# kostas1515/object_detectors

Hardware: AMD Instinct MI355X
Metric: images/sec (fwd+bwd) YOLOv3 640px bs=32 (higher is better)
Workload: dtype bf16; 1 GPU; YOLOv3 Darknet-53 training step (fwd+loss+bwd+SGD step), synthetic COCO 640px, per-GPU bs=32, 7 GT/img, random-init weights; global_batch=32, parallelism=dp1

## Files before the change

### object_detectors_amd/build.py

```python
import os
import subprocess
import sys
from concurrent.futures import ThreadPoolExecutor

HERE = os.path.dirname(os.path.abspath(__file__))
CSRC = os.path.join(HERE, "csrc")
OBJ = os.path.join(CSRC, "build")
LIB = os.path.join(HERE, "libmi355det.so")
HIPCC = os.environ.get("HIPCC", "/opt/rocm/bin/hipcc")
ARCH = "gfx950"

SOURCES = [
    ("lib.cpp", []),
    ("yolo_kernels.hip", ["-ffp-contract=off"]),
    ("box_kernels.hip", ["-ffp-contract=off"]),
    ("roi_kernels.hip", ["-ffp-contract=off"]),
    ("proposal_kernels.hip", ["-ffp-contract=off"]),
    ("frcnn_kernels.hip", ["-ffp-contract=off"]),
    ("transform_kernels.hip", ["-ffp-contract=off"]),
    ("mask_kernels.hip", ["-ffp-contract=off"]),
    ("resnet_kernels.hip", []),
    ("conv_kernels.hip", []),
    ("igemm8_kernels.hip", []),
    ("wgrad_kernels.hip", []),
    ("dgrad_s2_kernels.hip", []),
    ("elem_kernels.hip", []),
    ("stem_kernels.hip", ["-fno-slp-vectorize"]),
    ("stem_l1_kernels.hip", ["-fno-slp-vectorize"]),
    ("rstem_kernels.hip", ["-fno-slp-vectorize"]),
]
F16_TWINS = ["conv_kernels.hip", "igemm8_kernels.hip", "wgrad_kernels.hip", "dgrad_s2_kernels.hip", "elem_kernels.hip", "stem_kernels.hip",
             "stem_l1_kernels.hip"]
COMMON = ["-O3", "-std=c++17", "-fPIC", f"--offload-arch={ARCH}", "-Wno-unused-value", "-x", "hip"]


def _stale(out, deps):
    if not os.path.exists(out):
        return True
    t = os.path.getmtime(out)
    return any(os.path.getmtime(d) > t for d in deps)


def build(force=False, verbose=False):
    os.makedirs(OBJ, exist_ok=True)
    headers = [os.path.join(CSRC, f) for f in os.listdir(CSRC) if f.endswith(".h")]
    headers.append(os.path.join(HERE, "..", "include", "mi355det.h"))
    jobs, objs = [], []
    for src, extra in SOURCES:
        sp = os.path.join(CSRC, src)
        if not os.path.exists(sp):
            raise FileNotFoundError(sp)
        op = os.path.join(OBJ, os.path.splitext(src)[0] + ".o")
        objs.append(op)
        if force or _stale(op, [sp] + headers):
            jobs.append([HIPCC] + COMMON + extra + ["-c", sp, "-o", op])
        if src in F16_TWINS:
            op16 = os.path.join(OBJ, os.path.splitext(src)[0] + "_f16.o")
            objs.append(op16)
            if force or _stale(op16, [sp] + headers):
                jobs.append([HIPCC] + COMMON + extra + ["-DMI355_F16=1", "-c", sp, "-o", op16])

    def run(cmd):
        if verbose:
            print(" ".join(cmd), flush=True)
# ... 15 lines not shown
```

### object_detectors_amd/csrc/conv_kernels.hip

```cpp
#include "common.h"

#include <cstdlib>

#include <unordered_map>

#include "tune_record.h"

using namespace mi355;

#include "igemm_common.h"

extern int g_wgrad_general;
extern int g_wgrad_force_dbg;
extern int g_wgrad8_off;
extern int g_wgrad_ablate;
extern int g_dgrad_s2_off;
extern int g_conv_strict;
int mi355det_internal_dgrad_s2(const mi355det_conv_shape* s, const void* dy, const void* wt, void* dx, const void* residual, int32_t residual_ld,
                               void* stream, int probe = 0);

namespace {

#define STAMP(v) do { if (PROF) { __builtin_amdgcn_sched_barrier(0); asm volatile("s_memtime %0\n\ts_waitcnt lgkmcnt(0)" : "=s"(v) :: "memory"); __builtin_amdgcn_sched_barrier(0); } } while (0)

template <int WM, int WN, int TM, int TN, int BK, int NST, int EPI, bool PROF = false, bool ILV = false, int OCC = 0, int ABL = 0>
__global__ __launch_bounds__(WM* WN * 64, (OCC > 0 ? OCC : (WM * WN >= 8 ? 2 : 1))) void igemm_kernel(const IgemmParams p) {
  unsigned long long t_a = 0, t_b = 0, t_c = 0, t_d = 0, t_e = 0, c_wait = 0, c_bar = 0, c_issue = 0, c_comp = 0, t_begin = 0, t_loop = 0;
  STAMP(t_begin);
  constexpr int NT = WM * WN * 64;
  constexpr int NW = WM * WN;
  constexpr int BM = WM * TM * 16, BN = WN * TN * 16;
  constexpr int ROWB = BK * 2;
  constexpr int R = 1024 / ROWB;
  constexpr int CPR = BK / 8;
  constexpr int A_INSTR = BM / R, B_INSTR = BN / R;
  constexpr int A_PER = (A_INSTR + NW - 1) / NW, B_PER = (B_INSTR + NW - 1) / NW;
  constexpr int PER = A_PER + B_PER;
  constexpr int STAGE = (BM + BN) * ROWB;
  constexpr int D = NST - 1;
  static_assert(A_INSTR % NW == 0, "A tile must split evenly over the waves");
  extern __shared__ __attribute__((aligned(16))) char smem[];
  int* s_toff = (int*)(smem + NST * STAGE);

  const int tid = threadIdx.x, lane = tid & 63;
  const int wid = __builtin_amdgcn_readfirstlane(tid >> 6);
  const int wm = wid % WM, wn = wid / WM;

// ... 947 lines not shown
    if (ms < best_ms) {
      best_ms = ms;
      best = cfg;
    }
  }
  g_igemm_tuned[igemm_key(p, EPI)] = best;
  tune_mark_timed(TUNE_IGEMM, igemm_key(p, EPI));
  static const bool tune_log = getenv("MI355DET_TUNE_LOG") != nullptr;
  if (tune_log) fprintf(stderr, "[mi355det] igemm tune: M=%d Cout=%d Cin=%d T=%d epi=%d -> cfg %d (%.1f us)\n", p.M, p.CoutPad, p.Cin, p.T, EPI, best, best_ms * 1e3f / 3.f);
  return best;
}

__global__ __launch_bounds__(256) void lattice_fill_kernel(bf16_t* __restrict__ dx, int ld, const bf16_t* __restrict__ res, int ldres, int n, int h, int w,
                                                            int mh, int mw, int py, int px, int c) {
  const int c8 = c / 8;
  const long long total = (long long)n * mh * mw * c8;
  for (long long i = (long long)blockIdx.x * blockDim.x + threadIdx.x; i < total; i += (long long)gridDim.x * blockDim.x) {
    const int ch = (int)(i % c8);
    long long t = i / c8;
    const int xx = (int)(t % mw);
    t /= mw;
    const int yy = (int)(t % mh), im = (int)(t / mh);
    const int oy = 2 * yy + py, ox = 2 * xx + px;
    if (oy >= h || ox >= w) continue;
    const long long pix = ((long long)im * h + oy) * w + ox;
    uint4 v = make_uint4(0, 0, 0, 0);
    if (res) v = *(const uint4*)(res + pix * ldres + ch * 8);
    *(uint4*)(dx + pix * ld + ch * 8) = v;
  }
}

bool g_autotune_mode = false;
TuneMap& g_s2cat_tuned = tune_table(TUNE_S2CAT);
int g_s2cat_force = -1;

template <int EPI>
int dispatch_igemm(const IgemmParams& p_in, hipStream_t st) {
  IgemmParams p = p_in;
  p.lin_in = p.T == 1 && p.dy[0] == 0 && p.dx[0] == 0 && p.sin == 1 && p.MH == p.Hin && p.MW == p.Win;
  p.lin_out = p.so == 1 && p.sox == 0 && p.oy0 == 0 && p.ox0 == 0 && p.MH == p.Hout && p.MW == p.Wout;
  return g_autotune_mode ? autotune_igemm<EPI>(p, st) : launch_igemm<EPI>(p, st);
}

void set_tap_pad(IgemmParams& p) {
  int mn = 0;
  p.dy_pack = p.dx_pack = 0;
  for (int t = 0; t < p.T; ++t) {
    mn = min(mn, (p.dy[t] * p.Win + p.dx[t]) * p.ldin);
    p.dy_pack |= (unsigned long long)(p.dy[t] + 2) << (4 * t);
    p.dx_pack |= (unsigned long long)(p.dx[t] + 2) << (4 * t);
  }
  p.tap_pad = -mn;
}

int check_shape(const mi355det_conv_shape* s, const char* what) {
  if (!s) return fail(MI355DET_EINVAL, "%s: null shape", what);
  if (!((s->ksize == 1 && s->pad == 0) || (s->ksize == 3 && s->pad == 1)) || (s->stride != 1 && s->stride != 2))
    return fail(MI355DET_EINVAL, "%s: only 1x1/p0 and 3x3/p1 with stride 1 or 2 are supported", what);
  if (s->ho != (s->h + 2 * s->pad - s->ksize) / s->stride + 1 || s->wo != (s->w + 2 * s->pad - s->ksize) / s->stride + 1)
    return fail(MI355DET_EINVAL, "%s: output size does not match the convolution geometry", what);
  if (s->in_ld < s->cin || s->out_ld < s->cout) return fail(MI355DET_EINVAL, "%s: pixel pitch smaller than channel count", what);
  return 0;
}

int grid_m_rows(const mi355det_conv_shape* s, int cout_pad) {
  (void)cout_pad;
  const int bm = 128;
  const long long M = (long long)s->n * s->ho * s->wo;
  return (int)((M + bm - 1) / bm);
}

}

extern "C" {

int mi355det_debug_set(int key, int value) {
  if (key == 0) g_tune = value;
  if (key == 1) g_wgrad_general = value;
  if (key == 2) g_dgrad_s2_off = value;
  if (key == 3) igemm8_set_dbg_mode(value);
  if (key == 8) g_wgrad8_off = value;
  if (key == 7) g_wgrad_force_dbg = value;
  if (key == 6) g_wgrad_ablate = value;
  if (key == 5) g_s2cat_force = value;
  if (key == 9) g_conv_strict = value;
  return 0;
}

int mi355det_conv_autotune_mode(int on) {
  g_autotune_mode = on != 0;
  return 0;
}

int mi355det_debug_ptr(int key, void* ptr) {
  if (key == 0) g_dbg = (unsigned long long*)ptr;
  if (key == 1) igemm8_set_dbg((unsigned long long*)ptr);
  return 0;
}

int mi355det_conv_stats_rows(const mi355det_conv_shape* s, int32_t cout_pad) {
  if (!s) return 0;
  return grid_m_rows(s, cout_pad);
}

static int conv_fwd_impl(const mi355det_conv_shape* s, const void* x, const void* w, const float* bias, void* y, int out_f32, float* stats,
                         int32_t cout_pad, const mi355det_conv_epilogue* ex, void* stream) {
  if (int e = check_shape(s, "conv_fwd")) return e;
  if (int e = ensure_zero_page()) return e;
  if (cout_pad < s->cout) return fail(MI355DET_EINVAL, "%s: cout_pad < cout", "conv_fwd");
  if (!out_f32 && (s->cout % 8)) return fail(MI355DET_EINVAL, "%s: 16-bit outputs need cout %% 8 == 0 (got %lld)", "conv_fwd", s->cout);
  IgemmParams p{};
  p.x = (const bf16_t*)x;
  p.w = (const bf16_t*)w;
  p.y = y;
  p.bias = bias;
  p.stats = stats;
  p.zero = g_zero_page;
// ... 555 lines not shown
```

### object_detectors_amd/csrc/f16_names.h

```cpp
#pragma once
#define mi355det_conv_autotune_mode mi355det_conv_autotune_mode_f16
#define mi355det_conv_dgrad mi355det_conv_dgrad_f16
#define mi355det_conv_dgrad_bn mi355det_conv_dgrad_bn_f16
#define mi355det_conv_dgrad_bn_rows mi355det_conv_dgrad_bn_rows_f16
#define mi355det_conv_dgrad_mask mi355det_conv_dgrad_mask_f16
#define mi355det_conv_dgrad_workspace mi355det_conv_dgrad_workspace_f16
#define mi355det_conv_dgrad_ws mi355det_conv_dgrad_ws_f16
#define mi355det_conv_fwd mi355det_conv_fwd_f16
#define mi355det_conv_fwd_ex mi355det_conv_fwd_ex_f16
#define mi355det_conv_stats_rows mi355det_conv_stats_rows_f16
#define mi355det_debug_ptr mi355det_debug_ptr_f16
#define mi355det_debug_set mi355det_debug_set_f16
#define mi355det_dgrad_pack_elems mi355det_dgrad_pack_elems_f16
#define mi355det_pack_table_build mi355det_pack_table_build_f16
#define mi355det_pack_table_bytes mi355det_pack_table_bytes_f16
#define mi355det_pack_weights mi355det_pack_weights_f16
#define mi355det_pack_weights_batched mi355det_pack_weights_batched_f16
#define mi355det_stem_im2col mi355det_stem_im2col_f16
#define mi355det_unpack_wgrad mi355det_unpack_wgrad_f16
#define mi355det_conv_wgrad mi355det_conv_wgrad_f16
#define mi355det_conv_wgrad_autotune mi355det_conv_wgrad_autotune_f16
#define mi355det_conv_wgrad_workspace mi355det_conv_wgrad_workspace_f16
#define mi355det_add_bf16 mi355det_add_bf16_f16
#define mi355det_bn_act_bwd_apply mi355det_bn_act_bwd_apply_f16
#define mi355det_bn_act_bwd_reduce mi355det_bn_act_bwd_reduce_f16
#define mi355det_bn_act_bwd_reduce_det mi355det_bn_act_bwd_reduce_det_f16
#define mi355det_bn_act_bwd_reduce_workspace mi355det_bn_act_bwd_reduce_workspace_f16
#define mi355det_bn_act_fwd mi355det_bn_act_fwd_f16
#define mi355det_nchw_f32_to_nhwc mi355det_nchw_f32_to_nhwc_f16
#define mi355det_nhwc_to_nchw_f32 mi355det_nhwc_to_nchw_f32_f16
#define mi355det_upsample2x_bwd mi355det_upsample2x_bwd_f16
#define mi355det_upsample2x_fwd mi355det_upsample2x_fwd_f16
#define mi355det_stem_bwd_apply_wgrad mi355det_stem_bwd_apply_wgrad_f16
#define mi355det_stem_bwd_finish mi355det_stem_bwd_finish_f16
#define mi355det_stem_bwd_fused mi355det_stem_bwd_fused_f16
#define mi355det_stem_bwd_reduce mi355det_stem_bwd_reduce_f16
#define mi355det_stem_fwd_apply mi355det_stem_fwd_apply_f16
#define mi355det_stem_fwd_stats mi355det_stem_fwd_stats_f16
#define mi355det_stem_rows mi355det_stem_rows_f16
#define mi355det_stem_l1_fwd mi355det_stem_l1_fwd_f16
#define mi355det_stem_l1_fwd_eval mi355det_stem_l1_fwd_eval_f16
#define mi355det_stem_l1_rows mi355det_stem_l1_rows_f16
#define mi355det_internal_dgrad_s2 mi355det_internal_dgrad_s2_f16
#define igemm8_launch igemm8_launch_f16
#define igemm8_set_dbg igemm8_set_dbg_f16
#define igemm8_applicable igemm8_applicable_f16
#define igemm8_set_dbg_mode igemm8_set_dbg_mode_f16
#define g_wgrad_general g_wgrad_general_f16
#define g_wgrad_force_dbg g_wgrad_force_dbg_f16
#define g_conv_strict g_conv_strict_f16
#define g_wgrad8_off g_wgrad8_off_f16
#define g_wgrad_ablate g_wgrad_ablate_f16
#define g_dgrad_s2_off g_dgrad_s2_off_f16
#define pack_batched_kernel pack_batched_kernel_f16
#define splitk_reduce_kernel splitk_reduce_kernel_f16
```

### object_detectors_amd/csrc/igemm_common.h

```cpp
#pragma once
#include "common.h"

using namespace mi355;

typedef __attribute__((ext_vector_type(4))) float f32x4_t;
typedef __attribute__((ext_vector_type(8))) unsigned short u16x8_t;

#define MAX_TAPS 9

struct FastDiv {
  unsigned mul, shift;
};
static FastDiv make_fastdiv(unsigned d) {
  FastDiv f;
  unsigned l = 0;
  while ((1ull << l) < d) ++l;
  f.shift = l;
  f.mul = (unsigned)(((1ull << 32) * ((1ull << l) - d)) / d + 1);
  return f;
}
__device__ __forceinline__ unsigned fdiv(unsigned n, const FastDiv f) { return (__umulhi(f.mul, n) + n) >> f.shift; }

struct IgemmParams {
  const bf16_t* x;
// ... 5 lines not shown
  long long ynstride;
  const bf16_t* z;
  const float* ss;
  int ldz;
  float slope;
  float* stats;
  const bf16_t* res;
  const bf16_t* zero;
  int M, MH, MW;
  int Hin, Win, ldin, Cin, sin;
  int Hout, Wout, ldout, so, oy0, ox0;
  int sox;
  int Cout, CoutPad, ldres;
  int T;
  int dy[MAX_TAPS], dx[MAX_TAPS];
  FastDiv dMW, dMH;
  int tap_pad;
  unsigned long long dy_pack, dx_pack;
  int ksplit;
  long long ysplit;
  int lin_in, lin_out;
  unsigned long long* dbg;
};

enum { EPI_STATS = 0, EPI_F32 = 1, EPI_RES = 2, EPI_PLAIN = 3, EPI_AFF = 4, EPI_BNRED = 5 };
#define EPI_LDS_OFF 4096
#define EPI_LDS_BYTES(nwaves) (EPI_LDS_OFF + (nwaves) * (64 * (8 * 16 * 2 + 16) + 256))

bool igemm8_applicable(const IgemmParams& p);
int igemm8_launch(int epi, const IgemmParams& p, hipStream_t st, int rows = 256);
void igemm8_set_dbg(unsigned long long* ptr);
void igemm8_set_dbg_mode(int mode);

namespace {

__device__ __forceinline__ void glds16(const void* gsrc, void* lds_dst_uniform) {
  __builtin_amdgcn_global_load_lds((const __attribute__((address_space(1))) void*)gsrc,
                                   (__attribute__((address_space(3))) void*)lds_dst_uniform, 16, 0, 0);
}

typedef __attribute__((ext_vector_type(4))) int srd_t;
__device__ __forceinline__ srd_t make_srd(const void* base, unsigned num_records) {
  const unsigned long long a = (unsigned long long)base;
  srd_t r;
  r[0] = (int)(unsigned)a;
  r[1] = (int)((unsigned)(a >> 32) & 0xFFFFu);
  r[2] = (int)num_records;
  r[3] = 0x00020000;
  return r;
}
__device__ __forceinline__ void bufld16(srd_t rsrc, const void* lds_dst_uniform, int voffset, int soffset) {
  const unsigned lds = (unsigned)(unsigned long long)(__attribute__((address_space(3))) const void*)lds_dst_uniform;
  asm volatile("s_mov_b32 m0, %0\n\ts_nop 0\n\tbuffer_load_dwordx4 %1, %2, %3 offen lds" ::"s"(lds), "v"(voffset), "s"(rsrc), "s"(soffset) : "memory");
}
#define OOB_VOFF ((int)0x80000000)

__device__ __forceinline__ float row16_sum(float v) {
  v += __builtin_bit_cast(float, __builtin_amdgcn_update_dpp(0, __builtin_bit_cast(int, v), 0xB1, 0xF, 0xF, true));
  v += __builtin_bit_cast(float, __builtin_amdgcn_update_dpp(0, __builtin_bit_cast(int, v), 0x4E, 0xF, 0xF, true));
  v += __builtin_bit_cast(float, __builtin_amdgcn_update_dpp(0, __builtin_bit_cast(int, v), 0x141, 0xF, 0xF, true));
  v += __builtin_bit_cast(float, __builtin_amdgcn_update_dpp(0, __builtin_bit_cast(int, v), 0x140, 0xF, 0xF, true));
  return v;
}

template <int BK>
__device__ __forceinline__ int swz(int row) {
// ... 307 lines not shown
```

### object_detectors_amd/csrc/wgrad_kernels.hip

```cpp
#include "common.h"

#include <cstdlib>
#include <unordered_map>

#include "tune_record.h"

using namespace mi355;

typedef __attribute__((ext_vector_type(4))) short s16x4_t;
typedef __attribute__((ext_vector_type(4))) float f32x4_t;

struct FastDiv {
  unsigned mul, shift, d;
};

static FastDiv make_fastdiv(unsigned d) {
  FastDiv f;
  f.d = d;
  unsigned l = 0;
  while ((1ull << l) < d) ++l;
  f.shift = l;
  f.mul = (unsigned)(((1ull << 32) * ((1ull << l) - d)) / d + 1);
  return f;
}
__device__ __forceinline__ unsigned fdiv(unsigned n, const FastDiv f) {
  const unsigned t = __umulhi(f.mul, n);
  return (t + n) >> f.shift;
}

struct WgradParams {
  const bf16_t* x;
  const bf16_t* dy;
  float* dw;
  float* slab;
  const bf16_t* zero;
  int M, Ho, Wo, H, W, ldx, lddy, Cin, Cout, stride, pad, ks, T, NP;
  int co_tiles, np_tiles, splits, chunk;
  int step_q, step_r;
  FastDiv dWo, dHo, dCin;
  int ablate;
};

int g_wgrad_ablate = 0;
int g_wgrad_general = 0;
int g_conv_strict = 0;
int g_wgrad_force_dbg = 0;
int g_wgrad8_off = 0;

namespace {

#define WG_BKP 64
#define WG_TILE 128
#define WG_ROWB 256

__device__ __forceinline__ void glds16(const void* gsrc, void* lds_dst_uniform) {
  __builtin_amdgcn_global_load_lds((const __attribute__((address_space(1))) void*)gsrc,
                                   (__attribute__((address_space(3))) void*)lds_dst_uniform, 16, 0, 0);
}

typedef __attribute__((ext_vector_type(4))) int srd_t;
__device__ __forceinline__ srd_t make_srd(const void* base, unsigned num_records) {
  const unsigned long long a = (unsigned long long)base;
  srd_t r;
  r[0] = (int)(unsigned)a;
  r[1] = (int)((unsigned)(a >> 32) & 0xFFFFu);
  r[2] = (int)num_records;
  r[3] = 0x00020000;
  return r;
}
__device__ __forceinline__ void bufld16(srd_t rsrc, const void* lds_dst_uniform, int voffset, int soffset) {
  const unsigned lds = (unsigned)(unsigned long long)(__attribute__((address_space(3))) const void*)lds_dst_uniform;
  asm volatile("s_mov_b32 m0, %0\n\ts_nop 0\n\tbuffer_load_dwordx4 %1, %2, %3 offen lds" ::"s"(lds), "v"(voffset), "s"(rsrc), "s"(soffset) : "memory");
}
#define OOB_VOFF ((int)0x80000000)

__device__ __forceinline__ int rowf(int row) { return (row & 3) | (((row >> 3) & 1) << 2); }

__device__ __forceinline__ st16x4_t lds_tr(const char* p) {
  s16x4_t v = __builtin_amdgcn_ds_read_tr16_b64_v4i16((__attribute__((address_space(3))) s16x4_t*)p);
// ... 522 lines not shown

  const int fr = lane & 15, fq = lane >> 4;
  const int nt128 = NT * 2 + wm;
  if (nt128 >= p.np_tiles) return;
  if (p.slab) {
    const int tiles = p.co_tiles * p.np_tiles;
#pragma unroll
    for (int a = 0; a < 4; ++a) {
      const int col = wn * 64 + (a >> 1) * 32 + (a & 1) * 16;
      const int ct128 = CT * 2 + (col >> 7);
      if (ct128 >= p.co_tiles) continue;
      float* dst = p.slab + ((size_t)split * tiles + (size_t)nt128 * p.co_tiles + ct128) * (WG_TILE * WG_TILE);
#pragma unroll
      for (int r = 0; r < 4; ++r)
#pragma unroll
        for (int b = 0; b < 8; ++b) dst[((col & 127) + fq * 4 + r) * WG_TILE + (b >> 2) * 64 + (b & 3) * 16 + fr] = acc[a][b][r];
    }
    return;
  }
#pragma unroll
  for (int a = 0; a < 4; ++a)
#pragma unroll
    for (int r = 0; r < 4; ++r) {
      const int co = co0 + wn * 64 + (a >> 1) * 32 + (a & 1) * 16 + fq * 4 + r;
      if (co >= p.Cout) continue;
#pragma unroll
      for (int b = 0; b < 8; ++b) {
        const int np = np0 + wm * 128 + (b >> 2) * 64 + (b & 3) * 16 + fr;
        if (np < p.NP) p.dw[(long long)co * p.NP + np] += acc[a][b][r];
      }
    }
}

__global__ __launch_bounds__(256) void wgrad_reduce_kernel(const float* __restrict__ slab, float* __restrict__ dw, int Cout, int NP, int co_tiles,
                                                           int np_tiles, int splits) {
  const int tiles = co_tiles * np_tiles;
  const long long total = (long long)Cout * (NP / 4);
  const size_t sstride = (size_t)tiles * (WG_TILE * WG_TILE);
  for (long long i = blockIdx.x * 256ll + threadIdx.x; i < total; i += (long long)gridDim.x * 256) {
    const int co = (int)(i / (NP / 4)), np = (int)(i - (long long)co * (NP / 4)) * 4;
    const int ct = co / WG_TILE, nt = np / WG_TILE;
    const int tile = nt * co_tiles + ct;
    const float* src = slab + (size_t)tile * (WG_TILE * WG_TILE) + (co - ct * WG_TILE) * WG_TILE + (np - nt * WG_TILE);
    float4 a = make_float4(0.f, 0.f, 0.f, 0.f);
    for (int s0 = blockIdx.y * 8; s0 < splits; s0 += gridDim.y * 8) {
      float4 v[8];
#pragma unroll
      for (int u = 0; u < 8; ++u) v[u] = s0 + u < splits ? *(const float4*)(src + (size_t)(s0 + u) * sstride) : make_float4(0.f, 0.f, 0.f, 0.f);
#pragma unroll
      for (int u = 0; u < 8; ++u) {
        a.x += v[u].x; a.y += v[u].y; a.z += v[u].z; a.w += v[u].w;
      }
    }
    float* d = dw + (long long)co * NP + np;
    if (gridDim.y == 1) {
      float4 o = *(const float4*)d;
      o.x += a.x; o.y += a.y; o.z += a.z; o.w += a.w;
      *(float4*)d = o;
    } else {
      atomicAdd(d + 0, a.x); atomicAdd(d + 1, a.y); atomicAdd(d + 2, a.z); atomicAdd(d + 3, a.w);
    }
  }
}

__global__ __launch_bounds__(256) void wgrad_reduce8_kernel(const float* __restrict__ slab, float* __restrict__ dw, int Cout, int NP, int co_tiles,
                                                            int np_tiles, int splits) {
// ... 176 lines not shown
}

TuneMap& g_wgrad_tuned = tune_table(TUNE_WGRAD);
int g_wgrad_force = 0;
constexpr int WG_FORM8 = 1 << 16;

unsigned long long wgrad_key(const mi355det_conv_shape* s) {
  unsigned long long k = (unsigned long long)(s->n * s->ho * s->wo);
  k = k * 4099 + s->cout;
  k = k * 4099 + s->cin;
  k = k * 17 + s->ksize * 4 + s->stride;
  k = k * 2 + MI355_F16;
  return k;
}

bool split_valid(int M, int sp) {
  const int chunk = ((M + sp - 1) / sp + WG_BKP - 1) / WG_BKP * WG_BKP;
  return (M + chunk - 1) / chunk == sp;
}

bf16_t* g_zero_page_w = nullptr;
int ensure_zero_page_w() {
  if (g_zero_page_w) return 0;
  void* p = nullptr;
  if (hipMalloc(&p, 4096) != hipSuccess || hipMemset(p, 0, 4096) != hipSuccess) return fail(MI355DET_ELAUNCH, "%s: zero page alloc failed", "wgrad");
  g_zero_page_w = (bf16_t*)p;
  return 0;
}

bool wgrad8_applicable(const mi355det_conv_shape* s) {
  const long long NP = (long long)s->ksize * s->ksize * s->cin;
  if (s->wo < 4 || WG_BKP / s->wo + 1 > s->ho || s->cout < 256 || NP < 256 || s->cin % 8 != 0) return false;
  return ((long long)s->n * s->h * s->w + (long long)s->pad * (s->w + 1)) * s->in_ld * 2 < 0x7FFFFFF0ll;
}

}

extern "C" {

size_t mi355det_conv_wgrad_workspace(const mi355det_conv_shape* s) {
  if (!s) return 0;
  const size_t tiles = (size_t)((s->cout + WG_TILE - 1) / WG_TILE) * (size_t)((s->ksize * s->ksize * s->cin + WG_TILE - 1) / WG_TILE);
  const size_t per_split = tiles * WG_TILE * WG_TILE * sizeof(float);
  size_t splits = 1024;
  while (splits > 3 && splits * per_split > ((size_t)128 << 20)) --splits;
  return splits * per_split;
}

int mi355det_conv_wgrad_autotune(const mi355det_conv_shape* s, const void* x, const void* dy, float* dw, void* workspace,
                                 size_t workspace_bytes, void* stream) {
  if (!s) return fail(MI355DET_EINVAL, "%s: null shape", "wgrad_autotune");
  if (tune_locked_has(TUNE_WGRAD, wgrad_key(s))) return g_wgrad_tuned[wgrad_key(s)];
  const int M = s->n * s->ho * s->wo;
  const size_t tiles = (size_t)((s->cout + WG_TILE - 1) / WG_TILE) * (size_t)((s->ksize * s->ksize * s->cin + WG_TILE - 1) / WG_TILE);
  const size_t per_split = tiles * WG_TILE * WG_TILE * sizeof(float);
  const int cands[] = {1, 2, 3, 4, 5, 6, 7, 8, 10, 12, 14, 16, 20, 24, 28, 32, 40, 48, 56, 64, 96, 128, 192, 256, 384, 512, 768, 1024};
  hipEvent_t e0, e1;
  if (hipEventCreate(&e0) != hipSuccess || hipEventCreate(&e1) != hipSuccess) return fail(MI355DET_ELAUNCH, "%s: event create failed", "wgrad_autotune");
  int best = -1;
  float best_ms = 1e30f;
  int tried[32], n_tried = 0;
  float tried_ms[32];
  for (int sp : cands) {
    if (sp > 1 && (sp * per_split > workspace_bytes || M / sp < 512 || (size_t)sp * tiles > 4096)) continue;
    if (!split_valid(M, sp)) continue;
    g_wgrad_force = sp;
// ... 118 lines not shown
    form8 = form8 && wgrad8_applicable(s);
    const size_t per_split = (size_t)tiles * WG_TILE * WG_TILE * sizeof(float);
    while (splits > 1 && (splits * per_split > workspace_bytes || !split_valid(p.M, splits))) --splits;
  }
  int chunk = (p.M + splits - 1) / splits;
  chunk = (chunk + WG_BKP - 1) / WG_BKP * WG_BKP;
  splits = (p.M + chunk - 1) / chunk;
  p.splits = splits;
  p.chunk = chunk;
  p.slab = nullptr;
  if (splits > 1) {
    const size_t need = (size_t)splits * tiles * WG_TILE * WG_TILE * sizeof(float);
    if (!workspace || workspace_bytes < need) return fail(MI355DET_EWORKSPACE, "%s: workspace too small (%lld bytes needed)", "conv_wgrad", (long long)need);
    if (p.NP % 4 != 0) return fail(MI355DET_EINVAL, "%s: k*k*Cin must be a multiple of 4", "conv_wgrad");
    p.slab = (float*)workspace;
  }
  p.step_q = WG_BKP / p.Wo;
  p.step_r = WG_BKP % p.Wo;
  p.dWo = make_fastdiv((unsigned)p.Wo);
  p.dHo = make_fastdiv((unsigned)p.Ho);
  p.dCin = make_fastdiv((unsigned)p.Cin);
  const int lds = 2 * 2 * WG_BKP * WG_ROWB;
  const int ci = p.Cout <= 32 ? 1 : (p.Cout <= 64 ? 2 : 4), cj = p.NP <= 32 ? 1 : (p.NP <= 64 ? 2 : 4);
  auto go = [&](auto kern) {
    (void)hipFuncSetAttribute((const void*)kern, hipFuncAttributeMaxDynamicSharedMemorySize, lds);
    hipLaunchKernelGGL(kern, dim3(tiles * splits), dim3(256), lds, S(stream), p);
  };
  const int grp4 = g_wgrad_general != 0 || p.Wo < 4 || WG_BKP / p.Wo + 1 > p.Ho ? 0 : (p.Wo % 16 == 0 ? 3 : (p.Wo % 4 == 0 ? 1 : 2));
  const bool fits =
                    ((long long)s->n * p.H * p.W + (long long)p.pad * (p.W + 1)) * p.ldx * 2 < 0x7FFFFFF0ll &&
                    (long long)chunk * p.lddy * 2 < 0x7FFFFFF0ll;
  if (form8 && !fits && g_conv_strict && g_wgrad_force <= 0 && (g_wgrad_force_dbg & WG_FORM8))
    return fail(MI355DET_EINVAL, "%s: the forced phase-staggered kernel does not fit the 31-bit offsets of this shape (strict mode, debug key 9)", "conv_wgrad");
  if (form8 && fits) {
    const int tiles8 = ((p.Cout + W8_TILE - 1) / W8_TILE) * ((p.NP + W8_TILE - 1) / W8_TILE);
    static DeviceOnce attr8;
    attr8.once([&] {
      (void)hipFuncSetAttribute((const void*)wgrad8_kernel<false>, hipFuncAttributeMaxDynamicSharedMemorySize, W8_LDS);
      (void)hipFuncSetAttribute((const void*)wgrad8_kernel<true>, hipFuncAttributeMaxDynamicSharedMemorySize, W8_LDS);
    });
    if (p.Wo % 4 == 0 && p.M % 4 == 0) hipLaunchKernelGGL(wgrad8_kernel<false>, dim3(tiles8 * splits), dim3(512), W8_LDS, S(stream), p);
    else hipLaunchKernelGGL(wgrad8_kernel<true>, dim3(tiles8 * splits), dim3(512), W8_LDS, S(stream), p);
  } else
#define WG_GO(a, b) (!fits || grp4 == 0 ? go(wgrad_kernel<a, b, 0>) : grp4 == 1 ? go(wgrad_kernel<a, b, 1>) : grp4 == 2 ? go(wgrad_kernel<a, b, 2>) : go(wgrad_kernel<a, b, 3>))
  switch (ci * 8 + cj) {
    case 1 * 8 + 1: WG_GO(1, 1); break;
    case 1 * 8 + 2: WG_GO(1, 2); break;
    case 1 * 8 + 4: WG_GO(1, 4); break;
    case 2 * 8 + 1: WG_GO(2, 1); break;
    case 2 * 8 + 2: WG_GO(2, 2); break;
    case 2 * 8 + 4: WG_GO(2, 4); break;
    case 4 * 8 + 1: WG_GO(4, 1); break;
    case 4 * 8 + 2: WG_GO(4, 2); break;
    default: WG_GO(4, 4); break;
  }
#undef WG_GO
  if (p.slab) {
    const long long total = (long long)p.Cout * (p.NP / 4);
    if (splits >= 8) {
      const int gx = (int)min((long long)4096, (total + 31) / 32);
      hipLaunchKernelGGL(wgrad_reduce8_kernel, dim3(gx), dim3(256), 0, S(stream), p.slab, dw, p.Cout, p.NP, p.co_tiles, p.np_tiles, splits);
    } else {
      const int gx = (int)min((long long)2048, (total + 255) / 256);
      hipLaunchKernelGGL(wgrad_reduce_kernel, dim3(gx, 1), dim3(256), 0, S(stream), p.slab, dw, p.Cout, p.NP, p.co_tiles, p.np_tiles, splits);
    }
  }
  if (dbias) {
// ... 20 lines not shown
```

Measured before the change: 1157 images/s.

## Add row-streaming 3x3 conv kernel with register-resident weights for small-channel layers

Adds a new implicit-GEMM kernel for 3x3 stride-1 convolutions with small channel counts. Each block keeps all of its filter weights in registers and streams input rows through an LDS ring buffer. Output rows are written one step late so stores overlap the next step's loads. By default it handles only the Cin=64, Cout=32 case at 320 width (the Darknet-53 first residual block), in both the forward and flipped-tap paths. BN statistics are reduced per strip into the existing row-partial layout. The aim is to cut redundant halo and input reloads in a bandwidth-bound layer, at the cost of low occupancy (one block per CU, large LDS footprint) and more code paths.

Result: no change. 1158 images/s, median of 4 (+0.1%).

```diff
diff --git a/object_detectors_amd/build.py b/object_detectors_amd/build.py
--- a/object_detectors_amd/build.py
+++ b/object_detectors_amd/build.py
@@ -22,6 +22,7 @@
     ("resnet_kernels.hip", []),
     ("conv_kernels.hip", []),
     ("igemm8_kernels.hip", []),
+    ("rowstream_kernels.hip", []),
     ("wgrad_kernels.hip", []),
     ("dgrad_s2_kernels.hip", []),
     ("elem_kernels.hip", []),
@@ -29,7 +30,7 @@
     ("stem_l1_kernels.hip", ["-fno-slp-vectorize"]),
     ("rstem_kernels.hip", ["-fno-slp-vectorize"]),
 ]
-F16_TWINS = ["conv_kernels.hip", "igemm8_kernels.hip", "wgrad_kernels.hip", "dgrad_s2_kernels.hip", "elem_kernels.hip", "stem_kernels.hip",
+F16_TWINS = ["conv_kernels.hip", "igemm8_kernels.hip", "rowstream_kernels.hip", "wgrad_kernels.hip", "dgrad_s2_kernels.hip", "elem_kernels.hip", "stem_kernels.hip",
              "stem_l1_kernels.hip"]
 COMMON = ["-O3", "-std=c++17", "-fPIC", f"--offload-arch={ARCH}", "-Wno-unused-value", "-x", "hip"]
 
diff --git a/object_detectors_amd/csrc/conv_kernels.hip b/object_detectors_amd/csrc/conv_kernels.hip
--- a/object_detectors_amd/csrc/conv_kernels.hip
+++ b/object_detectors_amd/csrc/conv_kernels.hip
@@ -1026,6 +1026,7 @@
 
 bool g_autotune_mode = false;
 TuneMap& g_s2cat_tuned = tune_table(TUNE_S2CAT);
+int g_rowstream_mode = 0;
 int g_s2cat_force = -1;
 
 template <int EPI>
@@ -1033,6 +1034,8 @@
   IgemmParams p = p_in;
   p.lin_in = p.T == 1 && p.dy[0] == 0 && p.dx[0] == 0 && p.sin == 1 && p.MH == p.Hin && p.MW == p.Win;
   p.lin_out = p.so == 1 && p.sox == 0 && p.oy0 == 0 && p.ox0 == 0 && p.MH == p.Hout && p.MW == p.Wout;
+  if ((EPI == EPI_STATS || EPI == EPI_PLAIN) && g_rowstream_mode != 1 && g_tune == 0 && rowstream_applicable(p, EPI, g_rowstream_mode >= 2))
+    return rowstream_launch(EPI, p, st, g_rowstream_mode >= 3 ? g_rowstream_mode - 2 : 0);
   return g_autotune_mode ? autotune_igemm<EPI>(p, st) : launch_igemm<EPI>(p, st);
 }
 
@@ -1077,6 +1080,7 @@
   if (key == 7) g_wgrad_force_dbg = value;
   if (key == 6) g_wgrad_ablate = value;
   if (key == 5) g_s2cat_force = value;
+  if (key == 10) g_rowstream_mode = value;
   if (key == 9) g_conv_strict = value;
   return 0;
 }
diff --git a/object_detectors_amd/csrc/f16_names.h b/object_detectors_amd/csrc/f16_names.h
--- a/object_detectors_amd/csrc/f16_names.h
+++ b/object_detectors_amd/csrc/f16_names.h
@@ -46,6 +46,8 @@
 #define igemm8_set_dbg igemm8_set_dbg_f16
 #define igemm8_applicable igemm8_applicable_f16
 #define igemm8_set_dbg_mode igemm8_set_dbg_mode_f16
+#define rowstream_applicable rowstream_applicable_f16
+#define rowstream_launch rowstream_launch_f16
 #define g_wgrad_general g_wgrad_general_f16
 #define g_wgrad_force_dbg g_wgrad_force_dbg_f16
 #define g_conv_strict g_conv_strict_f16
diff --git a/object_detectors_amd/csrc/igemm_common.h b/object_detectors_amd/csrc/igemm_common.h
--- a/object_detectors_amd/csrc/igemm_common.h
+++ b/object_detectors_amd/csrc/igemm_common.h
@@ -61,6 +61,9 @@
 void igemm8_set_dbg(unsigned long long* ptr);
 void igemm8_set_dbg_mode(int mode);
 
+bool rowstream_applicable(const IgemmParams& p, int epi, bool all = false);
+int rowstream_launch(int epi, const IgemmParams& p, hipStream_t st, int strip_rows = 0);
+
 namespace {
 
 __device__ __forceinline__ void glds16(const void* gsrc, void* lds_dst_uniform) {
diff --git a/object_detectors_amd/csrc/rowstream_kernels.hip b/object_detectors_amd/csrc/rowstream_kernels.hip
--- /dev/null
+++ b/object_detectors_amd/csrc/rowstream_kernels.hip
@@ -0,0 +1,296 @@
+#include "igemm_common.h"
+
+namespace {
+
+constexpr int RS_ROW_BYTES = 21 * 1024;
+constexpr int RS_PIECES = 21;
+constexpr int RS_WAVES = 4;
+constexpr int RS_TPW = 5;
+
+struct RowstreamParams {
+  const bf16_t* x;
+  const bf16_t* w;
+  bf16_t* y;
+  float* stats;
+  int N, H, W, ldin, ldout, Cout, CoutPad;
+  int R;
+  int nstrips, ncol, ncs;
+  int flip;
+  int M;
+};
+
+template <int CIN>
+__device__ __forceinline__ int rs_swz(int s) {
+  return CIN == 32 ? ((s >> 1) & 3) : (s & 7);
+}
+
+template <int CIN, int NWC, int PX, int EPI>
+__global__ __launch_bounds__(RS_WAVES * 64, 1) void rowstream_kernel(const RowstreamParams p) {
+  static_assert(CIN == 32 || CIN == 64, "one or two k-steps of 32 per tap");
+  static_assert(NWC % 32 == 0, "output channels in pairs of 16-row tiles");
+  static_assert(320 % PX == 0 && PX % 80 == 0, "a step is 320 pixels; a wave's five tiles lie in one row");
+  constexpr int PB = CIN * 2;
+  constexpr int CPP = PB / 16;
+  constexpr int KS = CIN / 32;
+  constexpr int NT = NWC / 16;
+  constexpr int NP = NT / 2;
+  constexpr int RS = 320 / PX;
+  constexpr int NR = 2 * RS + 2;
+  constexpr int TPR = PX / 16;
+  constexpr int NPW = (RS_PIECES + RS_WAVES - 1) / RS_WAVES;
+  static_assert((PX + 2) * PB <= RS_ROW_BYTES, "ring row pitch");
+  extern __shared__ __attribute__((aligned(16))) char smem[];
+
+  const int tid = threadIdx.x, lane = tid & 63;
+  const int wid = __builtin_amdgcn_readfirstlane(tid >> 6);
+  const int fr = lane & 15, fq = lane >> 4;
+
+  int bid = blockIdx.x;
+  const int cs = bid % p.ncs;
+  bid /= p.ncs;
+  const int cc = bid % p.ncol;
+  bid /= p.ncol;
+  const int strip = bid % p.nstrips;
+  const int n = bid / p.nstrips;
+  const int y0 = strip * p.R;
+  const int y1 = min(y0 + p.R, p.H);
+  const int x0 = cc * PX;
+  const int c0 = cs * NWC;
+  const int nsteps = (y1 - y0 + RS - 1) / RS;
+
+  st16x8_t wreg[NT][9 * KS];
+#pragma unroll
+  for (int i = 0; i < NT; ++i) {
+    const int co = c0 + (i >> 1) * 32 + (fr >> 2) * 8 + (i & 1) * 4 + (fr & 3);
+    const bf16_t* wrow = p.w + (long long)co * (9 * CIN) + fq * 8;
+#pragma unroll
+    for (int g = 0; g < 9; ++g) {
+      const int t = p.flip ? 8 - g : g;
+#pragma unroll
+      for (int kk = 0; kk < KS; ++kk) wreg[i][g * KS + kk] = __builtin_bit_cast(st16x8_t, *(const uint4*)(wrow + t * CIN + kk * 32));
+    }
+  }
+
+  const srd_t rsrc = make_srd(p.x + (long long)n * p.H * p.W * p.ldin, 0x7FFFFFF0u);
+  int dvoff[NPW];
+#pragma unroll
+  for (int i = 0; i < NPW; ++i) {
+    const int pc = wid + RS_WAVES * i;
+    const int b = pc * 1024 + lane * 16;
+    const int s = b / PB, q = (b % PB) >> 4;
+    const int xx = x0 - 1 + s;
+    dvoff[i] = (pc < RS_PIECES && s < PX + 2 && xx >= 0 && xx < p.W) ? (xx * p.ldin + ((q ^ rs_swz<CIN>(s)) << 3)) * 2 : OOB_VOFF;
+  }
+  const int rowpitch = p.W * p.ldin * 2;
+  auto issue_row = [&](int ri) {
+    const int yin = y0 - 1 + ri;
+    const bool in = yin >= 0 && yin < p.H;
+    char* dst = smem + (ri % NR) * RS_ROW_BYTES;
+    const int soff = in ? yin * rowpitch : 0;
+#pragma unroll
+    for (int i = 0; i < NPW; ++i)
+      if (wid + RS_WAVES * i < RS_PIECES) bufld16(rsrc, dst + (wid + RS_WAVES * i) * 1024, in ? dvoff[i] : OOB_VOFF, soff);
+  };
+
+  const int rr = (wid * RS_TPW) / TPR;
+  const int xt = ((wid * RS_TPW) % TPR) * 16;
+  int boff[RS_TPW][3];
+#pragma unroll
+  for (int j = 0; j < RS_TPW; ++j)
+#pragma unroll
+    for (int d = 0; d < 3; ++d) {
+      const int s = xt + j * 16 + fr + d;
+      boff[j][d] = s * PB + ((fq ^ rs_swz<CIN>(s)) << 4);
+    }
+  const long long yimg = (long long)n * p.H * p.W * p.ldout;
+  const int ooff = (x0 + xt + fr) * p.ldout + c0 + fq * 8;
+
+  float s1[EPI == EPI_STATS ? NT * 4 : 1], s2[EPI == EPI_STATS ? NT * 4 : 1];
+  if (EPI == EPI_STATS) {
+#pragma unroll
+    for (int k = 0; k < NT * 4; ++k) s1[k] = s2[k] = 0.f;
+  }
+
+  uint4 pend[RS_TPW][NP];
+  int pend_row = -1;
+
+#pragma unroll
+  for (int r = 0; r < RS + 2; ++r) issue_row(r);
+
+  for (int st = 0; st < nsteps; ++st) {
+    wait_vmcnt<0>();
+    __builtin_amdgcn_s_barrier();
+    if (pend_row >= 0) {
+      bf16_t* orow = p.y + yimg + (long long)pend_row * p.W * p.ldout + ooff;
+#pragma unroll
+      for (int j = 0; j < RS_TPW; ++j)
+#pragma unroll
+        for (int pr = 0; pr < NP; ++pr) *(uint4*)(orow + j * 16 * p.ldout + pr * 32) = pend[j][pr];
+    }
+    if (st + 1 < nsteps) {
+#pragma unroll
+      for (int r = 0; r < RS; ++r) issue_row((st + 1) * RS + 2 + r);
+    }
+
+    f32x4_t acc[RS_TPW][NT];
+#pragma unroll
+    for (int j = 0; j < RS_TPW; ++j)
+#pragma unroll
+      for (int i = 0; i < NT; ++i) acc[j][i] = {0.f, 0.f, 0.f, 0.f};
+#pragma unroll
+    for (int dyi = 0; dyi < 3; ++dyi) {
+      const char* rowb = smem + ((st * RS + rr + dyi) % NR) * RS_ROW_BYTES;
+#pragma unroll
+      for (int dxi = 0; dxi < 3; ++dxi) {
+#pragma unroll
+        for (int kk = 0; kk < KS; ++kk) {
+#pragma unroll
+          for (int j = 0; j < RS_TPW; ++j) {
+            const st16x8_t b = *(const st16x8_t*)(rowb + (boff[j][dxi] ^ (kk * 64)));
+#pragma unroll
+            for (int i = 0; i < NT; ++i) acc[j][i] = MI355_MFMA_16x16x32(wreg[i][(dyi * 3 + dxi) * KS + kk], b, acc[j][i]);
+          }
+        }
+      }
+    }
+
+    const int yo = y0 + st * RS + rr;
+    const bool live = yo < y1;
+    if (live) {
+#pragma unroll
+      for (int j = 0; j < RS_TPW; ++j)
+#pragma unroll
+        for (int pr = 0; pr < NP; ++pr) {
+          unsigned o[4];
+#pragma unroll
+          for (int hf = 0; hf < 2; ++hf) {
+            const f32x4_t v = acc[j][pr * 2 + hf];
+            const bf16_t r0 = f2s(v[0]), r1 = f2s(v[1]), r2 = f2s(v[2]), r3 = f2s(v[3]);
+            o[hf * 2 + 0] = (unsigned)r0 | ((unsigned)r1 << 16);
+            o[hf * 2 + 1] = (unsigned)r2 | ((unsigned)r3 << 16);
+            if (EPI == EPI_STATS) {
+              const bf16_t rv[4] = {r0, r1, r2, r3};
+#pragma unroll
+              for (int r = 0; r < 4; ++r) {
+                const float f = s2f(rv[r]);
+                s1[(pr * 2 + hf) * 4 + r] += f;
+                s2[(pr * 2 + hf) * 4 + r] += f * f;
+              }
+            }
+          }
+          pend[j][pr] = make_uint4(o[0], o[1], o[2], o[3]);
+        }
+    }
+    pend_row = live ? yo : -1;
+  }
+  if (pend_row >= 0) {
+    bf16_t* orow = p.y + yimg + (long long)pend_row * p.W * p.ldout + ooff;
+#pragma unroll
+    for (int j = 0; j < RS_TPW; ++j)
+#pragma unroll
+      for (int pr = 0; pr < NP; ++pr) *(uint4*)(orow + j * 16 * p.ldout + pr * 32) = pend[j][pr];
+  }
+
+  if (EPI == EPI_STATS) {
+    __builtin_amdgcn_s_barrier();
+    float* sred = (float*)smem;
+#pragma unroll
+    for (int i = 0; i < NT; ++i)
+#pragma unroll
+      for (int r = 0; r < 4; ++r) {
+        const float a1 = row16_sum(s1[i * 4 + r]), a2 = row16_sum(s2[i * 4 + r]);
+        if (fr == 0) {
+          const int c = (i >> 1) * 32 + fq * 8 + (i & 1) * 4 + r;
+          sred[(wid * NWC + c) * 2 + 0] = a1;
+          sred[(wid * NWC + c) * 2 + 1] = a2;
+        }
+      }
+    __syncthreads();
+    const int nrows = (p.M + 127) / 128;
+    const int first = (n * p.H + y0) * p.W, next = (n * p.H + y1) * p.W;
+    const int r0 = first >> 7, r1 = next >= p.M ? nrows : next >> 7;
+    for (int c = tid; c < NWC; c += RS_WAVES * 64) {
+      float a1 = 0.f, a2 = 0.f;
+#pragma unroll
+      for (int w = 0; w < RS_WAVES; ++w) {
+        a1 += sred[(w * NWC + c) * 2 + 0];
+        a2 += sred[(w * NWC + c) * 2 + 1];
+      }
+      for (int row = r0; row < r1; ++row) {
+        float* dst = p.stats + (long long)row * 2 * p.CoutPad;
+        dst[c0 + c] = row == r0 ? a1 : 0.f;
+        dst[p.CoutPad + c0 + c] = row == r0 ? a2 : 0.f;
+      }
+    }
+  }
+}
+
+template <int CIN, int NWC, int PX, int EPI>
+int rs_launch(const RowstreamParams& p, hipStream_t st) {
+  constexpr int RS = 320 / PX;
+  constexpr int LDS = (2 * RS + 2) * RS_ROW_BYTES;
+  static DeviceOnce once;
+  once.once([] { (void)hipFuncSetAttribute((const void*)rowstream_kernel<CIN, NWC, PX, EPI>, hipFuncAttributeMaxDynamicSharedMemorySize, LDS); });
+  const int grid = p.N * p.nstrips * p.ncol * p.ncs;
+  hipLaunchKernelGGL((rowstream_kernel<CIN, NWC, PX, EPI>), dim3(grid), dim3(RS_WAVES * 64), LDS, st, p);
+  return check_launch("conv_rowstream");
+}
+
+int rs_tap_order(const IgemmParams& p) {
+  if (p.T != 9) return -1;
+  bool fwd = true, bwd = true;
+  for (int t = 0; t < 9; ++t) {
+    fwd = fwd && p.dy[t] == t / 3 - 1 && p.dx[t] == t % 3 - 1;
+    bwd = bwd && p.dy[t] == 1 - t / 3 && p.dx[t] == 1 - t % 3;
+  }
+  return fwd ? 0 : bwd ? 1 : -1;
+}
+
+}
+
+bool rowstream_applicable(const IgemmParams& p, int epi, bool all) {
+  if (epi != EPI_STATS && epi != EPI_PLAIN) return false;
+  if (rs_tap_order(p) < 0 || p.sin != 1 || p.so != 1 || p.sox != 0 || p.oy0 != 0 || p.ox0 != 0) return false;
+  if (p.MH != p.Hin || p.MW != p.Win || p.MH != p.Hout || p.MW != p.Wout || p.Hin < 1) return false;
+  if (p.ksplit > 1 || p.res != nullptr) return false;
+  const bool a = p.Cin == 32 && p.Cout == 64 && p.Win == 320;
+  const bool b = p.Cin == 64 && p.Cout == 32 && p.Win == 320;
+  const bool c = p.Cin == 64 && p.Cout == 128 && p.Win == 160;
+  if (!(b || (all && (a || c)))) return false;
+  if (p.CoutPad < p.Cout) return false;
+  if (p.ldin % 8 != 0 || p.ldout % 8 != 0 || p.ldin < p.Cin || p.ldout < p.Cout) return false;
+  if ((((unsigned long long)p.x) | ((unsigned long long)p.y) | ((unsigned long long)p.w)) & 15ull) return false;
+  if ((long long)p.Hin * p.Win * p.ldin * 2 >= (1ll << 30) || (long long)p.Hin * p.Win * p.ldout * 2 >= (1ll << 31)) return false;
+  if ((long long)p.M >= (1ll << 31) - 256) return false;
+  return true;
+}
+
+int rowstream_launch(int epi, const IgemmParams& q, hipStream_t st, int strip_rows) {
+  if (!rowstream_applicable(q, epi, true)) return fail(MI355DET_EINVAL, "%s: shape outside the row-streaming predicate", "conv_rowstream");
+  if (epi == EPI_STATS && !q.stats) return fail(MI355DET_EINVAL, "%s: null statistics buffer", "conv_rowstream");
+  RowstreamParams p{};
+  p.x = q.x;
+  p.w = q.w;
+  p.y = (bf16_t*)q.y;
+  p.stats = q.stats;
+  p.N = q.M / (q.MH * q.MW);
+  p.H = q.Hin;
+  p.W = q.Win;
+  p.ldin = q.ldin;
+  p.ldout = q.ldout;
+  p.Cout = q.Cout;
+  p.CoutPad = q.CoutPad;
+  p.flip = rs_tap_order(q);
+  p.M = q.M;
+  const int nwc = q.Cin == 32 ? 64 : 32, px = q.Cin == 32 ? 320 : 160, rs = 320 / px;
+  p.ncol = p.W / px;
+  p.ncs = p.Cout / nwc;
+  const int per_img = p.ncol * p.ncs;
+  int strips = (768 + p.N * per_img - 1) / (p.N * per_img);
+  const int max_strips = (p.H + rs - 1) / rs;
+  strips = strips < 1 ? 1 : strips > max_strips ? max_strips : strips;
+  p.R = ((strip_rows > 0 ? strip_rows : (p.H + strips - 1) / strips) + rs - 1) / rs * rs;
+  p.nstrips = (p.H + p.R - 1) / p.R;
+  if (q.Cin == 32) return epi == EPI_STATS ? rs_launch<32, 64, 320, EPI_STATS>(p, st) : rs_launch<32, 64, 320, EPI_PLAIN>(p, st);
+  return epi == EPI_STATS ? rs_launch<64, 32, 160, EPI_STATS>(p, st) : rs_launch<64, 32, 160, EPI_PLAIN>(p, st);
+}
```

## Add specialized narrow wgrad kernel for 3x3 Cin=32 Cout=64 convolutions

Applied to the files above, without the earlier changes.

Adds a dedicated weight-gradient kernel for 3x3, pad-1 convolutions with 32 input and 64 output channels. One workgroup covers the whole 64x288 weight tile per split, staging dy and all nine tap-shifted input slices into double-buffered LDS and running MFMA over them. It replaces the generic 128x128-tile wgrad path, which wastes most of its tile on this small shape. The new kernel is on by default, can be disabled through a new debug key, and applies only to the early-layer shape in Darknet-53.

Result: no change. 1142 images/s before, 1146 images/s after (median of 6 runs) (+0.3%).

```diff
diff --git a/object_detectors_amd/csrc/conv_kernels.hip b/object_detectors_amd/csrc/conv_kernels.hip
--- a/object_detectors_amd/csrc/conv_kernels.hip
+++ b/object_detectors_amd/csrc/conv_kernels.hip
@@ -13,6 +13,7 @@
 extern int g_wgrad_general;
 extern int g_wgrad_force_dbg;
 extern int g_wgrad8_off;
+extern int g_wgrad_narrow;
 extern int g_wgrad_ablate;
 extern int g_dgrad_s2_off;
 extern int g_conv_strict;
@@ -1077,6 +1078,7 @@
   if (key == 7) g_wgrad_force_dbg = value;
   if (key == 6) g_wgrad_ablate = value;
   if (key == 5) g_s2cat_force = value;
+  if (key == 10) g_wgrad_narrow = value;
   if (key == 9) g_conv_strict = value;
   return 0;
 }
diff --git a/object_detectors_amd/csrc/f16_names.h b/object_detectors_amd/csrc/f16_names.h
--- a/object_detectors_amd/csrc/f16_names.h
+++ b/object_detectors_amd/csrc/f16_names.h
@@ -50,6 +50,7 @@
 #define g_wgrad_force_dbg g_wgrad_force_dbg_f16
 #define g_conv_strict g_conv_strict_f16
 #define g_wgrad8_off g_wgrad8_off_f16
+#define g_wgrad_narrow g_wgrad_narrow_f16
 #define g_wgrad_ablate g_wgrad_ablate_f16
 #define g_dgrad_s2_off g_dgrad_s2_off_f16
 #define pack_batched_kernel pack_batched_kernel_f16
diff --git a/object_detectors_amd/csrc/wgrad_kernels.hip b/object_detectors_amd/csrc/wgrad_kernels.hip
--- a/object_detectors_amd/csrc/wgrad_kernels.hip
+++ b/object_detectors_amd/csrc/wgrad_kernels.hip
@@ -45,6 +45,7 @@
 int g_wgrad_general = 0;
 int g_conv_strict = 0;
 int g_wgrad_force_dbg = 0;
+int g_wgrad_narrow = 0;
 int g_wgrad8_off = 0;
 
 namespace {
@@ -633,6 +634,169 @@
     }
 }
 
+constexpr int WN_CIN = 32, WN_COUT = 64, WN_TAPS = 9;
+constexpr int WN_DROW = WN_COUT * 2, WN_XROW = WN_CIN * 2;
+constexpr int WN_NF = WN_TAPS * WN_CIN / 16 / 2;
+constexpr int WN_KP = 32;
+
+template <int KP>
+__global__ __launch_bounds__(256, KP == 32 ? 3 : 1) void wgradn_kernel(const WgradParams p) {
+  constexpr int D_BYTES = KP * WN_DROW, XT_BYTES = KP * WN_XROW, STAGE = D_BYTES + WN_TAPS * XT_BYTES;
+  constexpr int NPG = KP / 16;
+  constexpr int WPG = 4 / NPG;
+  constexpr int ND = KP / 32;
+  extern __shared__ __attribute__((aligned(16))) char smem[];
+  const int tid = threadIdx.x, lane = tid & 63;
+  const int wid = __builtin_amdgcn_readfirstlane(tid >> 6);
+  const int wr = wid & 1, wc = wid >> 1;
+
+  int split = blockIdx.x;
+  {
+    const int nblk = gridDim.x, q = nblk / 8, r = nblk % 8, xcd = split % 8, loc = split / 8;
+    split = (xcd < r ? xcd * (q + 1) : r * (q + 1) + (xcd - r) * q) + loc;
+  }
+  const int mA = split * p.chunk, mB = min(p.M, mA + p.chunk);
+  if (mA >= mB) return;
+
+  const int pg = wid % NPG, tsel = wid / NPG;
+  const int l16 = lane >> 2, xc = lane & 3;
+  const int xchunk = (((xc >> 1) ^ ((lane >> 5) & 1)) << 1) | (xc & 1);
+  const int lcx = (l16 * p.stride * p.ldx + xchunk * 8) * 2;
+  const int cxl = l16 * p.stride - p.pad;
+  int dyv[ND];
+#pragma unroll
+  for (int i = 0; i < ND; ++i) {
+    const int row = (wid * ND + i) * 8 + (lane >> 3), c = lane & 7;
+    const int f2 = ((row >> 1) & 1) | (((row >> 3) & 1) << 1);
+    dyv[i] = (row * p.lddy + ((((c >> 1) ^ f2) << 1) | (c & 1)) * 8) * 2;
+  }
+  const srd_t rsrc_x = make_srd(p.x - (p.pad * p.W + p.pad) * p.ldx, 0x7FFFFFF0u);
+  const int WoS = p.Wo * p.stride, HoS = p.Ho * p.stride;
+  const int c_ws = (KP % p.Wo) * p.stride, c_hs = (KP / p.Wo) * p.stride;
+  const int c_sb = (c_hs * p.W + c_ws) * p.ldx * 2;
+  const int c_row = (p.stride * p.W - WoS) * p.ldx * 2;
+  const int c_img = (p.H - HoS) * p.W * p.ldx * 2;
+  int g_hs, g_ws, g_sb;
+  {
+    const unsigned um = (unsigned)(mA + pg * 16);
+    const unsigned q1 = fdiv(um, p.dWo);
+    const int wo = (int)(um - q1 * p.Wo);
+    const unsigned n = fdiv(q1, p.dHo);
+    const int ho = (int)(q1 - n * p.Ho);
+    g_hs = ho * p.stride;
+    g_ws = wo * p.stride;
+    g_sb = (((int)n * p.H + g_hs) * p.W + g_ws) * p.ldx * 2;
+  }
+  auto stage = [&](int m_base, int buf) {
+    char* sd = smem + buf * STAGE;
+    char* sx = sd + D_BYTES;
+    const int rem = mB - m_base;
+    const srd_t rsrc_dy = make_srd(p.dy + (long long)m_base * p.lddy, (unsigned)(rem * p.lddy * 2));
+#pragma unroll
+    for (int i = 0; i < ND; ++i) bufld16(rsrc_dy, sd + (wid * ND + i) * 1024, dyv[i], 0);
+    const bool alive = pg * 16 < rem;
+#pragma unroll
+    for (int t = 0; t < WN_TAPS; ++t) {
+      if (WPG > 1 && t % WPG != tsel) continue;
+      const int kh = t / 3, kw = t % 3;
+      const bool ok = alive && (unsigned)(g_hs + kh - p.pad) < (unsigned)p.H && (unsigned)(g_ws + cxl + kw) < (unsigned)p.W;
+      bufld16(rsrc_x, sx + t * XT_BYTES + pg * 1024, ok ? lcx : OOB_VOFF, g_sb + (kh * p.W + kw) * p.ldx * 2);
+    }
+    g_ws += c_ws;
+    g_hs += c_hs;
+    g_sb += c_sb;
+    if (g_ws >= WoS) {
+      g_ws -= WoS;
+      g_hs += p.stride;
+      g_sb += c_row;
+    }
+    if (g_hs >= HoS) {
+      g_hs -= HoS;
+      g_sb += c_img;
+    }
+  };
+
+  f32x4_t acc[2][WN_NF];
+#pragma unroll
+  for (int i = 0; i < 2; ++i)
+#pragma unroll
+    for (int j = 0; j < WN_NF; ++j) acc[i][j] = {0.f, 0.f, 0.f, 0.f};
+
+  const int ksteps = (mB - mA + KP - 1) / KP;
+  stage(mA, 0);
+  asm volatile("s_waitcnt vmcnt(0)" ::: "memory");
+  __syncthreads();
+
+  const int g = lane >> 4, q = (lane & 15) >> 2, pp = lane & 3;
+  const int fd = ((q >> 1) & 1) | ((g & 1) << 1), fx = g & 1;
+  int ard[2], brd[WN_NF];
+#pragma unroll
+  for (int i = 0; i < 2; ++i) ard[i] = (8 * g + q) * WN_DROW + (((wr * 2 + i) ^ fd) << 5) + pp * 8;
+#pragma unroll
+  for (int j = 0; j < WN_NF; ++j) {
+    const int jj = wc * WN_NF + j;
+    brd[j] = D_BYTES + (jj >> 1) * XT_BYTES + (8 * g + q) * WN_XROW + (((jj & 1) ^ fx) << 5) + pp * 8;
+  }
+  for (int s = 0; s < ksteps; ++s) {
+    const int buf = s & 1;
+    if (s + 1 < ksteps) stage(mA + (s + 1) * KP, buf ^ 1);
+    const char* sb = smem + buf * STAGE;
+#pragma unroll
+    for (int ks = 0; ks < KP / 32; ++ks) {
+      st16x8_t af[2], bfr[WN_NF];
+#pragma unroll
+      for (int h = 0; h < 2; ++h) {
+        const int row = ks * 32 + 4 * h;
+#pragma unroll
+        for (int i = 0; i < 2; ++i) {
+          const st16x4_t v = lds_tr(sb + ard[i] + row * WN_DROW);
+          af[i][4 * h + 0] = v[0];
+          af[i][4 * h + 1] = v[1];
+          af[i][4 * h + 2] = v[2];
+          af[i][4 * h + 3] = v[3];
+        }
+#pragma unroll
+        for (int j = 0; j < WN_NF; ++j) {
+          const st16x4_t v = lds_tr(sb + brd[j] + row * WN_XROW);
+          bfr[j][4 * h + 0] = v[0];
+          bfr[j][4 * h + 1] = v[1];
+          bfr[j][4 * h + 2] = v[2];
+          bfr[j][4 * h + 3] = v[3];
+        }
+      }
+#pragma unroll
+      for (int i = 0; i < 2; ++i)
+#pragma unroll
+        for (int j = 0; j < WN_NF; ++j) acc[i][j] = MI355_MFMA_16x16x32(af[i], bfr[j], acc[i][j]);
+    }
+    asm volatile("s_waitcnt vmcnt(0)" ::: "memory");
+    __syncthreads();
+  }
+
+  const int fr = lane & 15, fq = lane >> 4;
+  if (p.slab) {
+    float* dst = p.slab + (size_t)split * (p.co_tiles * p.np_tiles) * (WG_TILE * WG_TILE);
+#pragma unroll
+    for (int i = 0; i < 2; ++i)
+#pragma unroll
+      for (int r = 0; r < 4; ++r)
+#pragma unroll
+        for (int j = 0; j < WN_NF; ++j) {
+          const int np = (wc * WN_NF + j) * 16 + fr;
+          dst[(size_t)((np >> 7) * p.co_tiles) * (WG_TILE * WG_TILE) + ((wr * 2 + i) * 16 + fq * 4 + r) * WG_TILE + (np & 127)] = acc[i][j][r];
+        }
+    return;
+  }
+#pragma unroll
+  for (int i = 0; i < 2; ++i)
+#pragma unroll
+    for (int r = 0; r < 4; ++r) {
+      const int co = (wr * 2 + i) * 16 + fq * 4 + r;
+#pragma unroll
+      for (int j = 0; j < WN_NF; ++j) p.dw[(long long)co * p.NP + (wc * WN_NF + j) * 16 + fr] += acc[i][j][r];
+    }
+}
+
 __global__ __launch_bounds__(256) void wgrad_reduce_kernel(const float* __restrict__ slab, float* __restrict__ dw, int Cout, int NP, int co_tiles,
                                                            int np_tiles, int splits) {
   const int tiles = co_tiles * np_tiles;
@@ -875,6 +1039,11 @@
   const long long NP = (long long)s->ksize * s->ksize * s->cin;
   if (s->wo < 4 || WG_BKP / s->wo + 1 > s->ho || s->cout < 256 || NP < 256 || s->cin % 8 != 0) return false;
   return ((long long)s->n * s->h * s->w + (long long)s->pad * (s->w + 1)) * s->in_ld * 2 < 0x7FFFFFF0ll;
+}
+
+bool wgrad_narrow_applicable(const mi355det_conv_shape* s) {
+  return s->ksize == 3 && s->pad == 1 && s->cin == WN_CIN && s->cout == WN_COUT && (s->stride == 1 || s->stride == 2) && s->wo % 16 == 0 &&
+         WG_BKP / s->wo + 1 <= s->ho;
 }
 
 }
@@ -1059,7 +1228,15 @@
                     (long long)chunk * p.lddy * 2 < 0x7FFFFFF0ll;
   if (form8 && !fits && g_conv_strict && g_wgrad_force <= 0 && (g_wgrad_force_dbg & WG_FORM8))
     return fail(MI355DET_EINVAL, "%s: the forced phase-staggered kernel does not fit the 31-bit offsets of this shape (strict mode, debug key 9)", "conv_wgrad");
-  if (form8 && fits) {
+  const bool narrow = g_wgrad_narrow != 1 && !p.ablate && !form8 && fits && wgrad_narrow_applicable(s) &&
+                      ((long long)s->n * p.H * p.W + 3ll * (p.W + 1)) * p.ldx * 2 < 0x7FFFFFF0ll;
+  if (narrow) {
+    auto gon = [&](auto kern, int bytes) {
+      (void)hipFuncSetAttribute((const void*)kern, hipFuncAttributeMaxDynamicSharedMemorySize, bytes);
+      hipLaunchKernelGGL(kern, dim3(splits), dim3(256), bytes, S(stream), p);
+    };
+    gon(wgradn_kernel<WN_KP>, 2 * WN_KP * (WN_DROW + WN_TAPS * WN_XROW));
+  } else if (form8 && fits) {
     const int tiles8 = ((p.Cout + W8_TILE - 1) / W8_TILE) * ((p.NP + W8_TILE - 1) / W8_TILE);
     static DeviceOnce attr8;
     attr8.once([&] {
```
